# m-hamza-mughal/convofusion

Hardware: AMD Instinct MI355X
Metric: denoise-steps/sec (B=32 per GPU, 196-token latent, 1500 audio tokens, 1000-step DDPM schedule) (higher is better)
Workload: dtype f16x3 (fp16 hi/lo split operands, 3 MFMAs per product, f32 accumulate; f32-equivalent); fused cross-attention against the long (audio) memory: single-f16 operands (keys, values, queries, probabilities), f32 accumulate, in DDPM runs (operand policy 15; 1000-step DDPM golden at this shape: 2.3e-5 from; 1 GPU; configs[1]: B=32/GPU synthetic, L=196, S=(32, 1500, 32, 8, 1), 7-way guidance (denoiser batch 224), DDPM 1000-step schedule, 20 timed iterations of the hipGraph-captured loop; parallelism=batch-shard x1, one all_gather of latents

## Files before the change

convofusion_amd/csrc/attn_fused.hpp:

```cpp
#pragma once
#include "cfd_common.hpp"

struct SelfAttnArgs {
  const char* qk;
  const char* vts;
  char* o;
  int L, Lv;
};

#define SELF_ATTN_WAVES 8
#define SA_WAIT_VM_LGKM0(N) __builtin_amdgcn_s_waitcnt(((N) & 15) | 0x70 | ((((N) >> 4) & 3) << 14))
template <int CFD_KI = 0>
__global__ void __launch_bounds__(SELF_ATTN_WAVES * 64, 4) self_attn_fused_kernel(const SelfAttnArgs a) {
  extern __shared__ __attribute__((aligned(16))) char smem[];
  constexpr int STAGE = 32768, VOFF = 16384;
  const int lane = threadIdx.x & 63;
  const int wid = __builtin_amdgcn_readfirstlane(threadIdx.x >> 6);
  const int l15 = lane & 15, q4 = lane >> 4, sw = l15 >> 1;
  const int b = blockIdx.z, h = blockIdx.y;
  const int q = blockIdx.x * (SELF_ATTN_WAVES * 16) + wid * 16 + l15;
  const bool qvalid = q < a.L;
  const bool wave_active = (int)(blockIdx.x * (SELF_ATTN_WAVES * 16)) + wid * 16 < a.L;
  const int qc = qvalid ? q : a.L - 1;
  const long long ROW = 4096;

  const int cpos = lane & 7, rsub = lane >> 3;
  const int nkv = (a.L + 31) / 32;
  auto fill = [&](int kt) __attribute__((always_inline)) {
    char* st = smem + (kt & 1) * STAGE;
#pragma unroll
    for (int n = 0; n < 2; ++n) {
      const int g = wid + SELF_ATTN_WAVES * n, ks = g >> 2, rg = g & 3;
      const int r = rg * 8 + rsub;
      const int key = min(kt * 32 + r, a.L - 1);
      const char* src = a.qk + ((long long)b * a.L + key) * ROW + (long long)(16 + h * 4 + ks) * 128 + ((cpos ^ ((r >> 1) & 7)) << 4);
      __builtin_amdgcn_global_load_lds((gptr_t)src, (lptr_t)(st + ks * 4096 + rg * 1024), 16, 0, 0);
    }
#pragma unroll
    for (int n = 0; n < 2; ++n) {
      const int rg = wid + SELF_ATTN_WAVES * n;
      const int r = rg * 8 + rsub;
      const char* src = a.vts + ((long long)b * CFD_D + h * 128 + r) * ((long long)a.Lv * 4) + (long long)kt * 128 + ((cpos ^ ((r >> 1) & 7)) << 4);
      __builtin_amdgcn_global_load_lds((gptr_t)src, (lptr_t)(st + VOFF + rg * 1024), 16, 0, 0);
    }
  };
  fill(0);

  spx8 qh[4], ql[4];
  {
    const char* qp = a.qk + ((long long)b * a.L + qc) * ROW + (long long)(h * 4) * 128 + q4 * 16;
#pragma unroll
    for (int ks = 0; ks < 4; ++ks) {
      qh[ks] = *reinterpret_cast<const spx8*>(qp + ks * 128);
      ql[ks] = *reinterpret_cast<const spx8*>(qp + ks * 128 + 64);
    }
  }
  f32x4 o[8];
#pragma unroll
  for (int f = 0; f < 8; ++f) o[f] = f32x4{0.f, 0.f, 0.f, 0.f};
  float m = -INFINITY, lsum = 0.f, mc_run = -INFINITY;

  for (int kt = 0; kt < nkv; ++kt) {
    SA_WAIT_VM_LGKM0(0);
    __builtin_amdgcn_s_barrier();
    if (kt + 1 < nkv) fill(kt + 1);
    if (!wave_active) continue;
    const char* st = smem + (kt & 1) * STAGE;

    f32x4 s[2];
#pragma unroll
    for (int t = 0; t < 2; ++t) s[t] = f32x4{0.f, 0.f, 0.f, 0.f};
#pragma unroll
    for (int ks = 0; ks < 4; ++ks) {
#pragma unroll
      for (int t = 0; t < 2; ++t) {
        const char* kp = st + ks * 4096 + (t * 16 + l15) * 128;
        const spx8 xh = *reinterpret_cast<const spx8*>(kp + ((q4 ^ sw) << 4));
        const spx8 xl = *reinterpret_cast<const spx8*>(kp + (((4 + q4) ^ sw) << 4));
        s[t] = SP_MFMA(xl, qh[ks], s[t], 0, 0, 0);
        s[t] = SP_MFMA(xh, ql[ks], s[t], 0, 0, 0);
        s[t] = SP_MFMA(xh, qh[ks], s[t], 0, 0, 0);
      }
    }
// ... 3 lines not shown
#pragma unroll
    for (int e = 0; e < 8; ++e) {
      const int key = kt * 32 + 16 * (e >> 2) + 4 * q4 + (e & 3);
      p[e] = key < a.L ? s[e >> 2][e & 3] : -INFINITY;
      mx = fmaxf(mx, p[e]);
    }
    mx = xlane_max(mx);
    const float m_new = fmaxf(m, mx);
    const float mc = m_new * LOG2E;
    const float scale = __builtin_amdgcn_exp2f(mc_run - mc);
    mc_run = mc;
    float ps = 0.f;
#pragma unroll
    for (int e = 0; e < 8; ++e) {
      p[e] = __builtin_amdgcn_exp2f(fmaf(p[e], LOG2E, -mc));
      ps += p[e];
    }
    lsum = lsum * scale + xlane_sum(ps);
    m = m_new;
    if (!__all(scale == 1.0f)) {
#pragma unroll
      for (int f = 0; f < 8; ++f) { o[f][0] *= scale; o[f][1] *= scale; o[f][2] *= scale; o[f][3] *= scale; }
    }
    spx8 ph, pl;
#pragma unroll
    for (int e = 0; e < 8; ++e) {
      sp_t hi, lo;
      split_f32(p[e], hi, lo);
      ph[e] = hi;
      pl[e] = lo;
    }
#pragma unroll
    for (int f = 0; f < 8; ++f) {
      const char* vp = st + VOFF + (f * 16 + l15) * 128;
      const spx8 xh = *reinterpret_cast<const spx8*>(vp + ((q4 ^ sw) << 4));
      const spx8 xl = *reinterpret_cast<const spx8*>(vp + (((4 + q4) ^ sw) << 4));
      o[f] = SP_MFMA(xl, ph, o[f], 0, 0, 0);
      o[f] = SP_MFMA(xh, pl, o[f], 0, 0, 0);
      o[f] = SP_MFMA(xh, ph, o[f], 0, 0, 0);
    }
  }
  __syncthreads();
  {
    constexpr int RS = 64 * 4 + 16;
    char* strip = smem + wid * (16 * RS);
    const float inv = 1.0f / lsum;
#pragma unroll
    for (int half = 0; half < 2; ++half) {
#pragma unroll
      for (int f = 0; f < 4; ++f) {
        const f32x4 src = o[half * 4 + f];
        *reinterpret_cast<f32x4*>(strip + l15 * RS + (f * 16 + q4 * 4) * 4) = f32x4{src[0] * inv, src[1] * inv, src[2] * inv, src[3] * inv};
      }
      asm volatile("s_waitcnt lgkmcnt(0)" ::: "memory");
#pragma unroll
      for (int it = 0; it < 2; ++it) {
        const int row = it * 8 + (lane >> 3), c8 = (lane & 7) * 8;
        const int qq = blockIdx.x * (SELF_ATTN_WAVES * 16) + wid * 16 + row;
        const f32x4 v0 = *reinterpret_cast<const f32x4*>(strip + row * RS + c8 * 4);
        const f32x4 v1 = *reinterpret_cast<const f32x4*>(strip + row * RS + c8 * 4 + 16);
        if (qq < a.L) {
          const float v[8] = {v0[0], v0[1], v0[2], v0[3], v1[0], v1[1], v1[2], v1[3]};
          sp_store8(a.o + ((long long)b * a.L + qq) * (CFD_D * 4), h * 128 + half * 64 + c8, v);
        }
      }
      asm volatile("s_waitcnt lgkmcnt(0)" ::: "memory");
    }
  }
}
// ... 1 lines not shown
```

convofusion_amd/csrc/cfd_core.hip:

```cpp
#include "cfd_internal.hpp"

static thread_local char g_err[1024] = "";
int fail(int code, const char* fmt, ...) {
  va_list ap;
  va_start(ap, fmt);
  vsnprintf(g_err, sizeof(g_err), fmt, ap);
  va_end(ap);
  return code;
}

extern "C" const char* cfd_last_error(void) { return g_err; }

static long long env_int(const char* name, long long dflt) {
  const char* v = getenv(name);
  return v ? atoll(v) : dflt;
}

#ifndef CFD_SOURCE_HASH
#define CFD_SOURCE_HASH "unknown"
#endif
static const char g_source_hash[] = "cfd-src-hash:" CFD_SOURCE_HASH;
extern "C" const char* cfd_source_hash(void) { return g_source_hash + 13; }

extern "C" int cfd_create(const cfd_config* cfg, cfd_handle* out) {
// ... 36 lines not shown
  (void)hipEventCreate(&c->pev[0]);
  (void)hipEventCreate(&c->pev[1]);
  if (hipStreamCreateWithFlags(&c->own_stream, hipStreamNonBlocking) != hipSuccess) { delete c; return fail(CFD_E_HIP, "stream create"); }
  *out = c;
  return CFD_OK;
}

extern "C" void cfd_destroy(cfd_handle c) {
  if (!c) return;
  (void)hipSetDevice(c->cfg.device);
  (void)hipDeviceSynchronize();
  if (c->gexec) (void)hipGraphExecDestroy(c->gexec);
  if (c->graph) (void)hipGraphDestroy(c->graph);
  for (auto& wg : c->weg_graph) {
    if (wg.exec) (void)hipGraphExecDestroy(wg.exec);
    if (wg.graph) (void)hipGraphDestroy(wg.graph);
  }
  if (c->weg_ev) (void)hipEventDestroy(c->weg_ev);
  c->weg_io.release();
  c->weg_rt_ws.release();
  c->sat.release();
  c->acen.release();
  for (auto& kv : c->raw) kv.second.release();
  DBuf* all[] = {&c->we_sp, &c->wp_sp, &c->wp_f, &c->ln_cd_p, &c->we_all, &c->be_all, &c->tsin, &c->weg_ws, &c->weg_tok, &c->latents, &c->coef, &c->inoise, &c->hist, &c->wtab, &c->esrc, &c->enoise, &c->ekeep};
  for (DBuf* b : all) b->release();
  c->wk[0].release();
  c->wk[1].release();
  for (int j = 0; j < CFD_NMEM; ++j) {
    c->wk_all_sp[j].release(); c->wv_all_sp[j].release(); c->mem_own[j].release(); c->perm_map[j].release();
    c->lv_map[j].release(); c->lv_mask[j].release();
  }
  c->pic_s.release(); c->pic_part.release(); c->pic_err.release();
  for (auto& l : c->lw) {
    DBuf* lb[] = {&l.wqk_f, &l.wv_f, &l.w1_f, &l.ln_cd, &l.wqk_sp, &l.bqk, &l.wv_sp, &l.wo_sp, &l.bo2, &l.wtb1_sp, &l.wtb2_sp, &l.w1_sp, &l.w2_sp, &l.cross_bias};
    for (DBuf* b : lb) b->release();
  }
  if (c->own_stream) (void)hipStreamDestroy(c->own_stream);
  if (c->pev[0]) (void)hipEventDestroy(c->pev[0]);
  if (c->pev[1]) (void)hipEventDestroy(c->pev[1]);
  delete c;
}

extern "C" int cfd_load_tensor(cfd_handle c, const char* name, const float* data, size_t numel, int is_device) {
  if (!c || !name || !data || numel == 0) return fail(CFD_E_ARG, "null/empty argument");
  HIPCHK(hipSetDevice(c->cfg.device));
  DBuf& b = c->raw[name];
  CHK(b.ensure(numel * sizeof(float)));
  HIPCHK(hipMemcpy(b.p, data, numel * sizeof(float), is_device ? hipMemcpyDeviceToDevice : hipMemcpyHostToDevice));
  c->raw_numel[name] = numel;
  c->finalized = false;
  c->weg_sig.clear();
  return CFD_OK;
}

static int need(Ctx* c, const std::string& name, size_t numel, const float** out, bool at_least = false) {
  auto it = c->raw_numel.find(name);
  if (it == c->raw_numel.end()) return fail(CFD_E_STATE, "missing tensor '%s' (state-dict key denoiser.%s)", name.c_str(), name.c_str());
  if (at_least ? (it->second < numel || it->second % CFD_D) : (it->second != numel))
    return fail(CFD_E_SHAPE, "tensor '%s' has %zu elements, expected %s%zu", name.c_str(), it->second, at_least ? ">= " : "", numel);
  *out = c->raw[name].as<float>();
  return CFD_OK;
}

int to_sp(Ctx* c, const float* src, long long R, int K, DBuf& dst, long long dst_rows) {
  if (dst_rows < 0) dst_rows = R;
  CHK(dst.ensure((size_t)dst_rows * K * 4));
  if (dst_rows > R) HIPCHK(hipMemset(dst.p, 0, (size_t)dst_rows * K * 4));
// ... 64 lines not shown
  CHK(c->be_all.ensure((size_t)nl * 2 * 2 * D * 4));
  DBuf tmpf, tmpd1, tmpd2, vd1, vd2, accd, tmpfold;
  CHK(tmpf.ensure((size_t)3 * D * D * 4));
  CHK(tmpd1.ensure((size_t)D * D * 8));
  CHK(tmpd2.ensure((size_t)D * D * 8));
  CHK(vd1.ensure(D * 8));
  CHK(vd2.ensure(D * 8));
  CHK(accd.ensure(D * 8));
  const long long kfeat = (long long)nl * D;
  DBuf wk_f[CFD_NMEM], wv_f[CFD_NMEM];
  for (int j = 0; j < CFD_NMEM; ++j) {
    CHK(wk_f[j].ensure((size_t)(kfeat + 32) * D * 4));
    HIPCHK(hipMemset(wk_f[j].p, 0, (size_t)(kfeat + 32) * D * 4));
    CHK(wv_f[j].ensure((size_t)kfeat * D * 4));
  }
  const dim3 blk(256);
  auto grid1 = [](long long n) { return dim3((unsigned)((n + 255) / 256)); };

  for (int l = 0; l < nl; ++l) {
    LayerW& w = c->lw[l];
    const std::string p = "decoder.layers." + std::to_string(l) + ".";
    const float *ipw, *ipb, *ow, *ob;
    const float* ipw_self = nullptr;
    CHK(need(c, p + "self_attn.in_proj_weight", (size_t)3 * D * D, &ipw));
    ipw_self = ipw;
    CHK(need(c, p + "self_attn.in_proj_bias", 3 * D, &ipb));
    CHK(need(c, p + "self_attn.out_proj.weight", (size_t)D * D, &ow));
    CHK(need(c, p + "self_attn.out_proj.bias", D, &ob));
    const float qs = (float)std::sqrt(1.0 / (double)CFD_HD);
    float* tf = tmpf.as<float>();
    hipLaunchKernelGGL(scale_copy_kernel<>, grid1((long long)D * D), blk, 0, 0, ipw, tf, (long long)D * D, qs);
    hipLaunchKernelGGL(scale_copy_kernel<>, grid1((long long)D * D), blk, 0, 0, ipw + (size_t)D * D, tf + (size_t)D * D,
                       (long long)D * D, 1.0f);
    CHK(to_sp(c, tf, 2 * D, D, w.wqk_sp));
    CHK(w.bqk.ensure(2 * D * 4));
    hipLaunchKernelGGL(scale_copy_kernel<>, grid1(D), blk, 0, 0, ipb, w.bqk.as<float>(), (long long)D, qs);
    hipLaunchKernelGGL(scale_copy_kernel<>, grid1(D), blk, 0, 0, ipb + D, w.bqk.as<float>() + D, (long long)D, 1.0f);
    CHK(to_sp(c, ipw + (size_t)2 * D * D, D, D, w.wv_sp));
    CHK(to_sp(c, ow, D, D, w.wo_sp));
    CHK(w.bo2.ensure(D * 4));
    hipLaunchKernelGGL((fold_mv_kernel<float, float, float>), grid1(D), blk, 0, 0, ow, (long long)D, 1LL, ipb + 2 * D,
                       (const double*)nullptr, ob, w.bo2.as<float>(), D, D, 1.0, (const float*)nullptr);
    for (int tb = 0; tb < 2; ++tb) {
      const std::string q = p + (tb == 0 ? "time_block1." : "time_block2.");
      CHK(need(c, q + "emb_layers.1.weight", (size_t)2 * D * D, &t0));
      HIPCHK(hipMemcpy(c->we_all.as<float>() + ((size_t)(2 * l + tb) * 2 * D) * D, t0, (size_t)2 * D * D * 4, hipMemcpyDeviceToDevice));
      CHK(need(c, q + "emb_layers.1.bias", 2 * D, &t0));
      HIPCHK(hipMemcpy(c->be_all.as<float>() + (size_t)(2 * l + tb) * 2 * D, t0, (size_t)2 * D * 4, hipMemcpyDeviceToDevice));
      CHK(need(c, q + "out_layers.2.weight", (size_t)D * D, &t0));
      CHK(to_sp(c, t0, D, D, tb == 0 ? w.wtb1_sp : w.wtb2_sp));
      CHK(need(c, q + "norm.weight", D, tb == 0 ? &w.tb1g : &w.tb2g));
      CHK(need(c, q + "norm.bias", D, tb == 0 ? &w.tb1b : &w.tb2b));
      CHK(need(c, q + "out_layers.2.bias", D, tb == 0 ? &w.btb1 : &w.btb2));
    }
    CHK(need(c, p + "norm1.weight", D, &w.ln1g)); CHK(need(c, p + "norm1.bias", D, &w.ln1b));
    CHK(need(c, p + "norm2.weight", D, &w.ln2g)); CHK(need(c, p + "norm2.bias", D, &w.ln2b));
    CHK(need(c, p + "norm3.weight", D, &w.ln3g)); CHK(need(c, p + "norm3.bias", D, &w.ln3b));
    CHK(need(c, p + "linear1.weight", (size_t)CFD_FF * D, &t0)); CHK(to_sp(c, t0, CFD_FF, D, w.w1_sp));
    CHK(need(c, p + "linear1.bias", CFD_FF, &w.b1));
    {
      CHK(w.ln_cd.ensure(6144 * 4));
      float* cd = w.ln_cd.as<float>();
      CHK(ln_fold_weight(c, tmpf.as<float>(), 2 * D, D, w.ln1g, w.ln1b, tmpfold, w.wqk_f, cd, cd + 1024));
      CHK(ln_fold_weight(c, ipw_self + (size_t)2 * D * D, D, D, w.ln1g, w.ln1b, tmpfold, w.wv_f, cd + 2048, cd + 2560));
      CHK(ln_fold_weight(c, t0, CFD_FF, D, w.ln3g, w.ln3b, tmpfold, w.w1_f, cd + 3072, cd + 4096));
    }
    CHK(need(c, p + "linear2.weight", (size_t)D * CFD_FF, &t0)); CHK(to_sp(c, t0, D, CFD_FF, w.w2_sp));
    CHK(need(c, p + "linear2.bias", D, &w.b2));
    const float *fw, *fb;
    CHK(need(c, p + "att_fuser.weight", (size_t)D * 5 * D, &fw));
    CHK(need(c, p + "att_fuser.bias", D, &fb));
// ... 67 lines not shown
```

convofusion_amd/csrc/cfd_forward.hip:

```cpp
#include "cfd_internal.hpp"



int enqueue_denoise(Ctx* c, hipStream_t st) {
  CHK(enqueue_memside(c, st));
  if (c->w->pb.rt) return enqueue_rows_rt(c, st);
  return enqueue_rows(c, st, 0, c->w->pb.Be);
}


int enqueue_rows_rt(Ctx* c, hipStream_t st, const RtSave* sv) {
  const Problem& p = c->w->pb;
  const int nl = c->nl, L = p.L, tpr = (L + 15) / 16, ntile = p.Be * tpr;
  const int* dstep = c->w->d_step.as<int>();
  const int lds_xpv = (p.Sp_tot / 32) * 2048 + 8 * (p.Sp_tot <= 512 ? 2 : 4) * 2048 + 16 * 32 * 16 + 512 + 2048;
#define RT_SET_LDS(kernel, bytes) HIPCHK(hipFuncSetAttribute(reinterpret_cast<const void*>(&kernel), hipFuncAttributeMaxDynamicSharedMemorySize, bytes))
  static unsigned long long attr = 0;
  if (!((attr >> (c->cfg.device & 63)) & 1ull)) {
    RT_SET_LDS((rt_gemm_kernel<RT_PRO_SP, RT_EPI_EMBED, 256, CFD_LAT / 32, 1>), rt_gemm_lds(RT_PRO_SP, 256, CFD_LAT / 32, 1));
    RT_SET_LDS((rt_gemm_kernel<RT_PRO_LN, RT_EPI_QKV, 512, CFD_D / 32, 3>), rt_gemm_lds(RT_PRO_LN, 512, CFD_D / 32, 3));
    RT_SET_LDS((rt_gemm_kernel<RT_PRO_SP, RT_EPI_RESID, 256, CFD_D / 32, 1>), rt_gemm_lds(RT_PRO_SP, 256, CFD_D / 32, 1));
    RT_SET_LDS((rt_gemm_kernel<RT_PRO_ADALN, RT_EPI_RESID, 512, CFD_D / 32, 1>), rt_gemm_lds(RT_PRO_ADALN, 512, CFD_D / 32, 1));
    RT_SET_LDS((rt_gemm_kernel<RT_PRO_LN, RT_EPI_SPLIT, 512, CFD_D / 32, 2>), rt_gemm_lds(RT_PRO_LN, 512, CFD_D / 32, 2));
    RT_SET_LDS((rt_gemm_kernel<RT_PRO_SP, RT_EPI_RESID, 512, CFD_FF / 32, 1>), rt_gemm_lds(RT_PRO_SP, 512, CFD_FF / 32, 1));
// ... 46 lines not shown
    if (_e != hipSuccess) return fail(CFD_E_HIP, "row-tile launch failed: %s", hipGetErrorString(_e));          \
  } while (0)
  {
    RtGemmArgs a = base;
    a.a_sp = c->w->sample_sp.as<char>(); a.w = c->we_sp.as<char>(); a.bias = rawp(c, "latent_embd.bias");
    a.bh = rawp(c, "bh_embedding.weight"); a.qpe = rawp(c, "query_pos.pe"); a.xo = X(0, 0);
    RT_LAUNCH(CFD_PROF_GEMM_TOKEN, RT_PRO_SP, RT_EPI_EMBED, 256, CFD_LAT / 32, 1, CFD_D, a);
  }
  if (c->stop_stage == 1) return CFD_OK;
  auto time_block = [&](const DBuf& w, const float* g, const float* b, const float* bias, int tbidx, const float* xin, float* xout) -> int {
    RtGemmArgs a = base;
    a.x = xin; a.xr = xin; a.xo = xout;
    a.g = g; a.b = b; a.ss = ss_now + (size_t)tbidx * 2 * CFD_D; a.w = w.as<char>(); a.bias = bias;
    if (nfb2) RT_LAUNCH(CFD_PROF_GEMM_TOKEN, RT_PRO_ADALN, RT_EPI_RESID, 512, CFD_D / 32, 2, CFD_D, a);
    else RT_LAUNCH(CFD_PROF_GEMM_TOKEN, RT_PRO_ADALN, RT_EPI_RESID, 512, CFD_D / 32, 1, CFD_D, a);
    return CFD_OK;
  };
  RtXArgs xa;
  memset(&xa, 0, sizeof(xa));
  xa.L = L; xa.tpr = tpr; xa.nl = nl; xa.Sp_tot = p.Sp_tot; xa.rsp = c->w->p_sp.as<float>();
  int nkb = 0;
  for (int j = 0; j < CFD_NMEM; ++j) {
    xa.map[j] = p.map[j]; xa.rows[j] = p.U[j] * p.Sp[j]; xa.S[j] = p.S[j]; xa.Sp[j] = p.Sp[j]; xa.off[j] = p.off[j];
    xa.cbt[j] = cbt_now[j]; xa.att[j] = p.att[j]; xa.att_slot[j] = p.att_slot[j];
    memcpy(xa.inst[j], p.rt_inst[j], RT_ARG_ROWS);
    xa.blk0[j] = nkb; nkb += p.Sp[j] / 16;
  }
  xa.blk0[CFD_NMEM] = nkb;
  xa.att_b0 = p.att_nb > 0 ? p.att_b0 : 0;
  xa.att_nb = p.att_nb > 0 ? p.att_nb : p.Be;
  xa.att_step = p.att_nb > 0 ? c->w->d_step.as<int>() : nullptr;
  for (int l = 0; l < nl; ++l) {
    const LayerW& w = c->lw[l];
    char* qk = sv ? sv->qk[l] : c->w->qk_sp.as<char>();
    char* vt = sv ? sv->vt[l] : c->w->rt_vt.as<char>();
    {
      RtGemmArgs a = base;
      a.x = X(l, 0);
      a.g = w.ln1g; a.b = w.ln1b; a.w = w.wqk_sp.as<char>(); a.w2 = w.wv_sp.as<char>(); a.nfb_qk = 2 * CFD_D / 16;
      a.bias = w.bqk.as<float>(); a.o_sp = qk; a.ld_o = 2 * CFD_D * 4; a.vt = vt;
      RT_LAUNCH(CFD_PROF_GEMM_TOKEN, RT_PRO_LN, RT_EPI_QKV, 512, CFD_D / 32, 3, 3 * CFD_D, a);
    }
    {
      RtSelfArgs a{qk, vt, c->w->o_sp.as<char>(), L, tpr};
      Bracket br(c, CFD_PROF_GEMM_ATTN, st);
      hipLaunchKernelGGL(rt_selfattn_kernel<>, dim3(CFD_NHEAD, ntile), dim3(256), 40960, st, a);
      HIPCHK(hipGetLastError());
    }
    {
      RtGemmArgs a = base;
      a.xr = X(l, 0); a.xo = X(l, 1);
      a.a_sp = c->w->o_sp.as<char>(); a.w = w.wo_sp.as<char>(); a.bias = w.bo2.as<float>();
      if (nfb2) RT_LAUNCH(CFD_PROF_GEMM_TOKEN, RT_PRO_SP, RT_EPI_RESID, 256, CFD_D / 32, 2, CFD_D, a);
      else RT_LAUNCH(CFD_PROF_GEMM_TOKEN, RT_PRO_SP, RT_EPI_RESID, 256, CFD_D / 32, 1, CFD_D, a);
    }
    if (c->stop_stage == 2 + 4 * l) return CFD_OK;
    CHK(time_block(w.wtb1_sp, w.tb1g, w.tb1b, w.btb1, 2 * l, X(l, 1), X(l, 2)));
    if (c->stop_stage == 3 + 4 * l) {
      if (!sv) HIPCHK(hipMemcpyAsync(xw, hw, (size_t)p.M * CFD_D * 4, hipMemcpyDeviceToDevice, st));
      return CFD_OK;
    }
    {
      RtXArgs a = xa;
      a.x = X(l, 2); a.xo = X(l, 3);
      a.sc = sv ? sv->sc[l] : c->w->sc.as<float>();
      a.cst = sv ? sv->cst[l] : c->w->ssc.as<float>();
      a.ln_g = w.ln2g; a.ln_b = w.ln2b; a.bias = w.cross_bias.as<float>(); a.layer = l;
      for (int j = 0; j < CFD_NMEM; ++j) {
        const size_t rows = (size_t)p.U[j] * p.Sp[j];
        a.K[j] = c->w->kall_sp[j].as<char>() + (size_t)l * rows * CFD_D * 4;
        a.VT[j] = c->w->vt_all[j].as<char>() + (size_t)l * rows * CFD_D * 4;
        a.kb[j] = kb_now[j] + (size_t)l * CFD_D;
// ... 113 lines not shown
  auto token_gemm_resid_ln = [&](const DBuf& w, int K, const char* y, const float* bias, long long rows, const float* g, const float* b,
                                 int adaln, int tbidx) -> int {
    CHK(token_gemm_resid(w, K, y, bias, rows));
    return ln(g, b, adaln, tbidx, c->w->h_sp.as<char>(), rows);
  };
  const bool ln_fold = c->ln_fold != 0 && L == 16 && !c->stop_stage && row0 == 0 && Be == p.Be &&
                       (c->ln_fold > 0 || (M >= 512 && M <= 3840));
  if (ln_fold) CHK(c->w->ln_stat.ensure((size_t)M * LN_SLOTS * 2 * 4));
  auto token_gemm_resid_stat = [&](const DBuf& w, int K, const char* y, const float* bias, long long rows, char* xs) -> int {
    GemmArgs a = gemm_args();
    a.X[0] = w.as<char>(); a.ldx[0] = (long long)K * 4; a.I[0] = CFD_D; a.Iclamp[0] = CFD_D; a.kt[0] = K / 32;
    a.Y = y; a.ldy = (long long)K * 4; a.J = (int)rows; a.Jclamp = (int)rows;
    EpiResidStat e{c->w->x.as<float>(), 0, bias, xs, c->w->ln_stat.as<float>()};
    return run_gemm_midsize<MODE_PLAIN>(c, CFD_PROF_GEMM_TOKEN, a, e, st);
  };
  bool h_raw = false;
  static unsigned long long attr = 0;
  if (!((attr >> (c->cfg.device & 63)) & 1ull)) {
    HIPCHK(hipFuncSetAttribute(reinterpret_cast<const void*>(&self_attn_fused_kernel<>), hipFuncAttributeMaxDynamicSharedMemorySize, 65536));
    HIPCHK(hipFuncSetAttribute(reinterpret_cast<const void*>(&xattn_fused_kernel<false, false>), hipFuncAttributeMaxDynamicSharedMemorySize, XA_LDS));
    HIPCHK(hipFuncSetAttribute(reinterpret_cast<const void*>(&xattn_fused_kernel<false, true>), hipFuncAttributeMaxDynamicSharedMemorySize, XA_LDS));
    HIPCHK(hipFuncSetAttribute(reinterpret_cast<const void*>(&xattn_fused_kernel<true, false>), hipFuncAttributeMaxDynamicSharedMemorySize, XA_LDS));
    attr |= 1ull << (c->cfg.device & 63);
  }

  bool h_ready = false;
  for (int l = 0; l < nl; ++l) {
    const LayerW& w = c->lw[l];
    const int Ba = (l == 0) ? Bs : Be;
    const long long Ma = (long long)Ba * L;
    if (!h_ready) CHK(ln(w.ln1g, w.ln1b, 0, 0, c->w->h_sp.as<char>(), Ma));
    h_ready = false;
    bool qkv_one_launch = false;
    const int Lv = (L + 31) / 32 * 32;
    {
      GemmArgs a = gemm_args();
      a.X[0] = w.wqk_sp.as<char>(); a.ldx[0] = ROWB; a.I[0] = 2 * CFD_D; a.Iclamp[0] = 2 * CFD_D; a.kt[0] = CFD_D / 32;
      a.Y = c->w->h_sp.as<char>(); a.ldy = ROWB; a.J = (int)Ma; a.Jclamp = (int)Ma;
      EpiSplit e{c->w->qk_sp.as<char>(), 2 * ROWB, 0, 0, w.bqk.as<float>(), 0, 0};
      GemmArgs av = gemm_args();
      av.X[0] = c->w->h_sp.as<char>(); av.ldx[0] = ROWB; av.xbs[0] = (long long)L * ROWB; av.I[0] = Lv; av.Iclamp[0] = L; av.kt[0] = CFD_D / 32;
      av.Y = w.wv_sp.as<char>(); av.ldy = ROWB; av.J = CFD_D; av.Jclamp = CFD_D;
      EpiSplit ev{c->w->vts_sp.as<char>(), (long long)Lv * 4, (long long)CFD_D * Lv * 4, 0, nullptr, 0, 1};
      if (L == 16) {
        GemmArgs ag = a;
        ag.nslot = 2;
        ag.X[1] = w.wv_sp.as<char>(); ag.ldx[1] = ROWB; ag.I[1] = CFD_D; ag.Iclamp[1] = CFD_D; ag.kt[1] = CFD_D / 32;
        EpiQkvT eg{c->w->qk_sp.as<char>(), 2 * ROWB, w.bqk.as<float>(), c->w->vts_sp.as<char>(), 1};
        if (h_raw) {
          EpiLn<EpiQkvT> el;
          static_cast<EpiQkvT&>(el) = eg;
          const float* cd = w.ln_cd.as<float>();
          el.ln_stat = c->w->ln_stat.as<float>(); el.ln_c[0] = cd; el.ln_d[0] = cd + 1024; el.ln_c[1] = cd + 2048; el.ln_d[1] = cd + 2560; el.ln_eps = 1e-5f;
          ag.X[0] = w.wqk_f.as<char>(); ag.X[1] = w.wv_f.as<char>();
          CHK((run_gemm_midsize<MODE_GROUPED>(c, CFD_PROF_GEMM_TOKEN, ag, el, st)));
        } else
        CHK((run_gemm<MODE_GROUPED>(c, CFD_PROF_GEMM_TOKEN, ag, eg, 1, 1, st)));
        qkv_one_launch = true;
      } else {
      CHK((run_gemm<MODE_PLAIN>(c, CFD_PROF_GEMM_TOKEN, a, e, 1, 1, st)));
      CHK((run_gemm<MODE_PLAIN>(c, CFD_PROF_GEMM_TOKEN, av, ev, Ba, 1, st)));
      }
    }
    if (qkv_one_launch) {
      RtSelfArgs a{c->w->qk_sp.as<char>(), c->w->vts_sp.as<char>(), c->w->o_sp.as<char>(), L, 1};
      Bracket br(c, CFD_PROF_GEMM_ATTN, st);
      hipLaunchKernelGGL(rt_selfattn_kernel<>, dim3(CFD_NHEAD, Ba), dim3(256), 40 * 1024, st, a);
      HIPCHK(hipGetLastError());
    } else {
      SelfAttnArgs a{c->w->qk_sp.as<char>(), c->w->vts_sp.as<char>(), c->w->o_sp.as<char>(), L, Lv};
      Bracket br(c, CFD_PROF_GEMM_ATTN, st);
      hipLaunchKernelGGL(self_attn_fused_kernel<>, dim3((L + SELF_ATTN_WAVES * 16 - 1) / (SELF_ATTN_WAVES * 16), CFD_NHEAD, Ba), dim3(SELF_ATTN_WAVES * 64), 65536, st, a);
      HIPCHK(hipGetLastError());
    }
    CHK(token_gemm_resid_ln(w.wo_sp, CFD_D, c->w->o_sp.as<char>(), w.bo2.as<float>(), Ma, w.tb1g, w.tb1b, 1, 2 * l));
    if (c->stop_stage == 2 + 4 * l) return CFD_OK;
    CHK(token_gemm_resid(w.wtb1_sp, CFD_D, c->w->h_sp.as<char>(), w.btb1, Ma));
    if (c->stop_stage == 3 + 4 * l) return CFD_OK;
    if (Ma != M) {
      const long long n4 = Ma * (CFD_D / 4);
      LAUNCH(CFD_PROF_ROWS, replicate_rows_kernel<>, dim3((unsigned)((n4 + 255) / 256)), blk, st, reinterpret_cast<float4*>(c->w->x.as<float>()), n4,
             (int)(M / Ma));
    }
    if (fused_x) {
      XAttnArgs a;
      memset(&a, 0, sizeof(a));
      a.x = c->w->x.as<float>(); a.ln_g = w.ln2g; a.ln_b = w.ln2b; a.bias = w.cross_bias.as<float>(); a.L = L;
      for (int j = 0; j < CFD_NMEM; ++j) {
        const size_t rows = (size_t)p.U[j] * p.Sp[j];
        const bool f16 = p.xa_f16 && ((p.xa_f16_mask >> j) & 1);
        a.K[j] = f16 ? c->w->k16[j].as<char>() + (size_t)l * rows * 1024 : c->w->kall_sp[j].as<char>() + (size_t)l * rows * ROWB;
        a.cb[j] = c->w->cb[j].as<float>() + (size_t)l * rows;
        a.VT[j] = f16 ? c->w->v16[j].as<char>() + (size_t)l * rows * 1024 : c->w->vt_all[j].as<char>() + (size_t)l * rows * ROWB;
        a.Sp[j] = p.Sp[j];
        const bool stat = (p.static_mask >> j) & 1;
        a.rs_off[j] = (unsigned)((size_t)(nl - l) * rows * 4);
        a.kb[j] = stat ? kb_now[j] + (size_t)l * CFD_D : c->w->zeros512.as<float>();
        a.kb_stride[j] = stat ? nl * CFD_D + 32 : 0;
        a.vb[j] = stat ? vb_now[j] + (size_t)l * CFD_D : c->w->zeros512.as<float>();
        a.vb_stride[j] = stat ? nl * CFD_D : 0;
      }
      a.d_step = rows_now ? nullptr : dstep;
      a.one_j = -1;
// ... 449 lines not shown
```

convofusion_amd/csrc/cfd_internal.hpp:

```cpp
#pragma once
#include <hip/hip_runtime.h>

#include <cmath>
#include <cstdarg>
#include <cstdio>
#include <cstdlib>
#include <cstring>
#include <algorithm>
#include <map>
#include <string>
#include <vector>

#include "../../include/cfdenoise.h"
#include "../../include/cfdenoise_dev.h"
#include "gemm_sp.hpp"
#include "rows.hpp"
#include "attn_fused.hpp"
#include "xattn_fused.hpp"
#include "rowtile.hpp"


int fail(int code, const char* fmt, ...);
#define HIPCHK(expr)                                                                               \
  do {                                                                                             \
    hipError_t _e = (expr);                                                                        \
    if (_e != hipSuccess) return fail(CFD_E_HIP, "%s failed: %s (%s:%d)", #expr, hipGetErrorString(_e), __FILE__, __LINE__); \
  } while (0)
#define CHK(expr)            \
  do {                       \
    int _r = (expr);         \
    if (_r != CFD_OK) return _r; \
  } while (0)

static const char* MEM_NAMES[CFD_NMEM] = {"spkemb", "alsn", "tlsn", "apb", "lsnemb"};

struct DBuf {
  void* p = nullptr;
  size_t bytes = 0;
  int ensure(size_t n) {
    if (n <= bytes) return CFD_OK;
    if (p) (void)hipFree(p);
    p = nullptr;
    bytes = 0;
    HIPCHK(hipMalloc(&p, n));
    bytes = n;
    return CFD_OK;
  }
  void release() {
    if (p) (void)hipFree(p);
    p = nullptr;
    bytes = 0;
  }
  template <class T> T* as() const { return reinterpret_cast<T*>(p); }
};

struct LayerW {
  DBuf wqk_sp, bqk, wv_sp, wo_sp, bo2, wtb1_sp, wtb2_sp, w1_sp, w2_sp, cross_bias;
  DBuf wqk_f, wv_f, w1_f, ln_cd;
  const float *ln1g, *ln1b, *tb1g, *tb1b, *btb1, *ln2g, *ln2b, *tb2g, *tb2b, *btb2, *ln3g, *ln3b, *b1, *b2;
};

struct Problem {
  int Be = 0, L = 0, Lp = 0;
  long long M = 0;
  int U[CFD_NMEM], S[CFD_NMEM], Sp[CFD_NMEM], off[CFD_NMEM], Sp_tot = 0;
  const float* mem[CFD_NMEM];
  const int* map[CFD_NMEM];
  const uint8_t* mask[CFD_NMEM];
  int has_mask[CFD_NMEM];
  float* att[CFD_NMEM];
  int att_b0 = 0, att_nb = 0;
  bool prev_same = false;
  bool att_fused = false;
  long long att_slot[CFD_NMEM] = {0, 0, 0, 0, 0};
  int tmode = 0;
  int lv_rows = 0, lv_i0 = 0, lv_U[CFD_NMEM] = {0, 0, 0, 0, 0};
  int share_B = 0;
  int T = 1;
  int jbig = -1, nruns = 0, nlong = 0, nshort = 0;
  int run_row0[8], run_len[8], run_u[8];
  int xa_nwg = 0;
  int xa0_nwg_a = 0, xa0_nwg_b = 0;
  bool xa_flush = false;
  int xa_one = -1;
  bool xa_f16 = false;
  int xa_f16_mask = 0;
  int static_mask = 0;
  bool rt = false;
  int rt_use_inst = 0;
  unsigned char rt_inst[CFD_NMEM][RT_ARG_ROWS];
};

struct RtSave {
  float* x[CFD_MAX_LAYERS + 1][5];
  char* qk[CFD_MAX_LAYERS];
  char* vt[CFD_MAX_LAYERS];
  float* sc[CFD_MAX_LAYERS];
  float* cst[CFD_MAX_LAYERS];
  float* pre[CFD_MAX_LAYERS];
};

struct WegRtState {
  std::vector<long long> sig;
  RtSave sv;
  float *att = nullptr, *d_att = nullptr, *fws = nullptr, *dP = nullptr, *G[3] = {nullptr, nullptr, nullptr}, *dz = nullptr, *dy = nullptr,
        *dh = nullptr, *dO = nullptr, *dqkv = nullptr;
  int launches = 0;
  int T = 1;
  int stop = 0, stop_gi = -1;
  int B = 0, L = 0, Sp_tot = 0, St = 0;
  int dy_keys = 0, focus_large = 0;
};

struct Work {
  Problem pb;
  DBuf x, h_sp, qk_sp, vts_sp, ssc, sp_sp, o_sp, u_sp, sc, p_sp, eps, sample_sp;
  DBuf ln_stat;
  DBuf n_sp[CFD_NMEM], kall_sp[CFD_NMEM], cb[CFD_NMEM], vt_all[CFD_NMEM];
  DBuf temb_tab, h1_tab, ss_tab, trows, iota, long_rows, short_rows, zero_mask;
  DBuf ca[CFD_NMEM], asq[CFD_NMEM], kbtab[CFD_NMEM], vbtab[CFD_NMEM], b_tab, b_sp, bsq, zeros512;
  DBuf xa_wgs, xa_segs, xa_stamps, xa0_wgs_a, xa0_segs_a, xa0_wgs_b, xa0_segs_b, xa_dedup, xa_one_va, xa_att_raw, xa_att_mc, xa_att_fin, xa_att_desc;
  DBuf d_step;
  bool fwd_mem_valid = false;
  int fwd_U[CFD_NMEM] = {0, 0, 0, 0, 0}, fwd_S[CFD_NMEM] = {0, 0, 0, 0, 0}, fwd_Be = 0, fwd_L = 0;
  bool fwd_att = false;
  bool fwd_mask[CFD_NMEM] = {false, false, false, false, false}, fwd_map[CFD_NMEM] = {false, false, false, false, false};
  unsigned long long fwd_wver = 0;
  DBuf rt_vt, rt_cbt[CFD_NMEM];
  DBuf k16[CFD_NMEM], v16[CFD_NMEM];
  DBuf rt_cur;
  std::vector<int32_t> tt_key;
  long long tt_wver = -1;
  int tt_mem_mask = 0;
  const float* now_ss = nullptr;
  const float* now_kb[CFD_NMEM] = {nullptr, nullptr, nullptr, nullptr, nullptr};
  const float* now_vb[CFD_NMEM] = {nullptr, nullptr, nullptr, nullptr, nullptr};
  void release() {
    DBuf* all[] = {&x, &h_sp, &qk_sp, &vts_sp, &ssc, &sp_sp, &o_sp, &u_sp, &sc, &p_sp, &eps, &sample_sp, &temb_tab, &h1_tab, &ss_tab, &trows, &iota,
                   &long_rows, &short_rows, &zero_mask, &ln_stat, &b_tab, &b_sp, &bsq, &zeros512, &xa_wgs, &xa_segs, &xa_stamps, &xa0_wgs_a, &xa0_segs_a, &xa0_wgs_b, &xa0_segs_b, &xa_dedup, &xa_one_va, &xa_att_raw, &xa_att_mc, &xa_att_fin, &xa_att_desc, &d_step, &rt_vt, &rt_cur};
    for (DBuf* b : all) b->release();
    for (int j = 0; j < CFD_NMEM; ++j) {
      n_sp[j].release(); kall_sp[j].release(); cb[j].release(); vt_all[j].release(); ca[j].release(); asq[j].release(); kbtab[j].release();
      vbtab[j].release(); rt_cbt[j].release(); k16[j].release(); v16[j].release();
    }
  }
};

struct RunMode {
  bool weighted = false;
  int k0 = 0;
  bool edit = false;
  float* traj = nullptr;
  bool anchor = false;
  const float* anchor_ring = nullptr;
  int anchor_n = 0;
  bool tie = false;
  bool tie_final = false;
  bool replay = false;
};

struct cfd_handle_s {
  cfd_config cfg;
  int nl = 0;
  bool finalized = false;
  std::map<std::string, DBuf> raw;
  std::map<std::string, size_t> raw_numel;
  DBuf we_sp, wp_sp, we_all, be_all;
  DBuf wp_f, ln_cd_p;
  DBuf wk_all_sp[CFD_NMEM], wv_all_sp[CFD_NMEM];
  std::vector<LayerW> lw;
  int qpe_rows = 0, mpe_rows = 0;
// ... 213 lines not shown
```

convofusion_amd/csrc/cfd_problem.hip:

```cpp
#include "cfd_internal.hpp"

struct XaRow {
  int xrow;
  int inst[CFD_NMEM];
  int aux;
  int one;
  int att;
};

static void make_xattn_worklist(const Problem& p, const std::vector<XaRow>& rows, int mem_mask, std::vector<XaWg>& wgs, std::vector<XaSeg>& segs,
                                size_t& n_active, bool& has_flush) {
  const int L = p.L, nqt = (L + 15) / 16;
  wgs.clear(); segs.clear(); n_active = 0;
  int order[CFD_NMEM], n_mem = 0, n_online = 0;
  for (int j = 0; j < CFD_NMEM; ++j)
    if ((mem_mask >> j) & 1) order[n_mem++] = j;
  if (n_mem == 0 || rows.empty()) return;
  std::stable_sort(order, order + n_mem, [&](int a, int b) { return p.Sp[a] > p.Sp[b]; });
  for (int oi = 0; oi < n_mem; ++oi) n_online += p.Sp[order[oi]] > XA_KEYS;
  const int jg = order[0];
  std::vector<int> inst_group(p.U[jg], -1);
  std::vector<std::vector<int>> groups;
  for (size_t r = 0; r < rows.size(); ++r) {
    int& g = inst_group[rows[r].inst[jg]];
// ... 287 lines not shown
        if (!srows.empty()) HIPCHK(hipMemcpy(c->w->short_rows.p, srows.data(), srows.size() * 4, hipMemcpyHostToDevice));
      }
    }
  }
  p.rt = c->rt_on && tmode == 0 && L <= RT_MAX_L && p.M <= c->rt_max_rows && p.Sp_tot <= RT_MAX_KEYS;
  if (p.rt) {
    if (!keep_lists) p.rt_use_inst = Be <= RT_ARG_ROWS;
    for (int j = 0; j < CFD_NMEM && p.rt_use_inst && !keep_lists; ++j) {
      std::vector<int> hm(Be);
      if (mem[j].row_map) HIPCHK(hipMemcpy(hm.data(), mem[j].row_map, (size_t)Be * 4, hipMemcpyDeviceToHost));
      else for (int b = 0; b < Be; ++b) hm[b] = b;
      for (int b = 0; b < Be; ++b) {
        if (hm[b] < 0 || hm[b] >= p.U[j]) return fail(CFD_E_ARG, "memory %s: row_map[%d] = %d outside [0, %d)", MEM_NAMES[j], b, hm[b], p.U[j]);
        if (hm[b] > 255) p.rt_use_inst = 0;
        p.rt_inst[j][b] = (unsigned char)hm[b];
      }
    }
    CHK(c->w->rt_vt.ensure((size_t)Be * CFD_D * RT_MAX_L * 4));
    HIPCHK(hipMemset(c->w->rt_vt.p, 0, (size_t)Be * CFD_D * RT_MAX_L * 4));
  }
  {
    bool any_att = false;
    for (int j = 0; j < CFD_NMEM; ++j) any_att = any_att || p.att[j];
    p.att_fused = any_att && !p.rt && tmode == 0 && c->fused_xattn;
    if (p.att_fused) { p.att_b0 = 0; p.att_nb = Be; }
  }
  if (!keep_lists) CHK(build_xattn_worklist(c, mem, true));
  if (p.att_fused && p.xa_nwg <= 0) { p.att_fused = false; p.att_nb = 0; }
  if (p.att_fused && !keep_lists) CHK(setup_att_fused(c));
  const long long M = p.M;
  const int nl = c->nl;
  CHK(c->w->x.ensure((size_t)M * CFD_D * 4));
  CHK(c->w->h_sp.ensure((size_t)M * CFD_D * 4));
  CHK(c->w->qk_sp.ensure((size_t)M * 2 * CFD_D * 4));
  CHK(c->w->vts_sp.ensure((size_t)Be * CFD_D * ((L + 63) / 64 * 64) * 4));
  CHK(c->w->ssc.ensure((size_t)Be * CFD_NHEAD * L * p.Lp * 4));
  CHK(c->w->sp_sp.ensure((size_t)Be * CFD_NHEAD * L * p.Lp * 4));
  CHK(c->w->o_sp.ensure((size_t)M * CFD_D * 4));
  CHK(c->w->u_sp.ensure((size_t)M * CFD_FF * 4));
  CHK(c->w->sc.ensure((size_t)M * p.Sp_tot * 4));
  CHK(c->w->p_sp.ensure((size_t)M * p.Sp_tot * 4));
  CHK(c->w->eps.ensure((size_t)M * CFD_LAT * 4));
  CHK(c->w->sample_sp.ensure((size_t)M * CFD_LAT * 4));
  for (int j = 0; j < CFD_NMEM; ++j) {
    const size_t rows = (size_t)p.U[j] * p.Sp[j];
    CHK(c->w->n_sp[j].ensure(rows * CFD_D * 4));
    CHK(c->w->kall_sp[j].ensure(rows * nl * CFD_D * 4));
    CHK(c->w->cb[j].ensure(rows * (nl + 1) * 4));
    CHK(c->w->vt_all[j].ensure(rows * nl * CFD_D * 4));
  }
  if (c->w->temb_tab.bytes < (size_t)T * CFD_D * 4 || c->w->ss_tab.bytes < (size_t)T * nl * 2 * 2 * CFD_D * 4) {
    c->w->tt_key.clear();
    c->w->tt_mem_mask = 0;
  }
  CHK(c->w->temb_tab.ensure((size_t)T * CFD_D * 4));
  CHK(c->w->h1_tab.ensure((size_t)T * CFD_D * 4));
  CHK(c->w->ss_tab.ensure((size_t)T * nl * 2 * 2 * CFD_D * 4));
  CHK(c->w->trows.ensure((size_t)T * 4));
  return CFD_OK;
}

int build_time_tables(Ctx* c, const int32_t* trows_host, int T, hipStream_t st) {
  for (int i = 0; i < T; ++i)
    if (trows_host[i] < 0 || trows_host[i] >= c->tsin_rows)
      return fail(CFD_E_ARG, "timestep %d outside the sinusoid table (0..%d)", trows_host[i], c->tsin_rows - 1);
  HIPCHK(hipMemcpyAsync(c->w->trows.p, trows_host, (size_t)T * 4, hipMemcpyHostToDevice, st));
  Work* w = c->w;
  const bool same = w->tt_wver == c->wver && (int)w->tt_key.size() == T && std::equal(w->tt_key.begin(), w->tt_key.end(), trows_host);
// ... 208 lines not shown
```

Baseline: 83.78 denoise-steps/s (32-utterance batches, summed over GPUs).

## Fuse V projection into QKV GEMM and read V via LDS transpose loads

Concatenates the Q, K and V projection weights into one weight so the token GEMM produces Q, K and V in a single row-major buffer. This removes the separate batched V-transpose GEMM launch. The self-attention kernel now loads V rows directly from that buffer and uses ds_read_tr16_b64 transpose reads from LDS to build the MFMA fragments. The cost is more complex swizzled LDS addressing and a wider QKV output row stride.

New measurement: 85.06 denoise-steps/s (32-utterance batches, summed over GPUs) (median of 6 runs). 1.02x the previous value.

```diff
diff --git a/convofusion_amd/csrc/attn_fused.hpp b/convofusion_amd/csrc/attn_fused.hpp
--- a/convofusion_amd/csrc/attn_fused.hpp
+++ b/convofusion_amd/csrc/attn_fused.hpp
@@ -2,11 +2,21 @@
 #include "cfd_common.hpp"
 
 struct SelfAttnArgs {
-  const char* qk;
-  const char* vts;
+  const char* qkv;
   char* o;
-  int L, Lv;
+  long long ldq;
+  int L;
 };
+
+typedef __fp16 sa_tr4 __attribute__((__vector_size__(4 * sizeof(__fp16))));
+__device__ __forceinline__ spx8 sa_tr_frag(const char* p) {
+  const sa_tr4 a = __builtin_amdgcn_ds_read_tr16_b64_v4f16((__attribute__((address_space(3))) sa_tr4*)(lptr_t)p);
+  const sa_tr4 b = __builtin_amdgcn_ds_read_tr16_b64_v4f16((__attribute__((address_space(3))) sa_tr4*)(lptr_t)(p + 2048));
+  spx8 r;
+#pragma unroll
+  for (int e = 0; e < 4; ++e) { r[e] = (sp_t)a[e]; r[4 + e] = (sp_t)b[e]; }
+  return r;
+}
 
 #define SELF_ATTN_WAVES 8
 #define SA_WAIT_VM_LGKM0(N) __builtin_amdgcn_s_waitcnt(((N) & 15) | 0x70 | ((((N) >> 4) & 3) << 14))
@@ -22,10 +32,11 @@
   const bool qvalid = q < a.L;
   const bool wave_active = (int)(blockIdx.x * (SELF_ATTN_WAVES * 16)) + wid * 16 < a.L;
   const int qc = qvalid ? q : a.L - 1;
-  const long long ROW = 4096;
+  const long long ROW = a.ldq;
 
   const int cpos = lane & 7, rsub = lane >> 3;
   const int nkv = (a.L + 31) / 32;
+  const int vpl = lane >> 5, vr = (lane >> 2) & 7, vch = vpl * 4 + ((((lane >> 1) & 1) ^ (vr >> 2)) << 1) + (lane & 1);
   auto fill = [&](int kt) __attribute__((always_inline)) {
     char* st = smem + (kt & 1) * STAGE;
 #pragma unroll
@@ -33,22 +44,22 @@
       const int g = wid + SELF_ATTN_WAVES * n, ks = g >> 2, rg = g & 3;
       const int r = rg * 8 + rsub;
       const int key = min(kt * 32 + r, a.L - 1);
-      const char* src = a.qk + ((long long)b * a.L + key) * ROW + (long long)(16 + h * 4 + ks) * 128 + ((cpos ^ ((r >> 1) & 7)) << 4);
+      const char* src = a.qkv + ((long long)b * a.L + key) * ROW + (long long)(16 + h * 4 + ks) * 128 + ((cpos ^ ((r >> 1) & 7)) << 4);
       __builtin_amdgcn_global_load_lds((gptr_t)src, (lptr_t)(st + ks * 4096 + rg * 1024), 16, 0, 0);
     }
 #pragma unroll
     for (int n = 0; n < 2; ++n) {
-      const int rg = wid + SELF_ATTN_WAVES * n;
-      const int r = rg * 8 + rsub;
-      const char* src = a.vts + ((long long)b * CFD_D + h * 128 + r) * ((long long)a.Lv * 4) + (long long)kt * 128 + ((cpos ^ ((r >> 1) & 7)) << 4);
-      __builtin_amdgcn_global_load_lds((gptr_t)src, (lptr_t)(st + VOFF + rg * 1024), 16, 0, 0);
+      const int g = wid + SELF_ATTN_WAVES * n, ks = g >> 2, rg = g & 3;
+      const int key = min(kt * 32 + rg * 8 + vr, a.L - 1);
+      const char* src = a.qkv + ((long long)b * a.L + key) * ROW + (long long)(32 + h * 4 + ks) * 128 + (vch << 4);
+      __builtin_amdgcn_global_load_lds((gptr_t)src, (lptr_t)(st + VOFF + g * 1024), 16, 0, 0);
     }
   };
   fill(0);
 
   spx8 qh[4], ql[4];
   {
-    const char* qp = a.qk + ((long long)b * a.L + qc) * ROW + (long long)(h * 4) * 128 + q4 * 16;
+    const char* qp = a.qkv + ((long long)b * a.L + qc) * ROW + (long long)(h * 4) * 128 + q4 * 16;
 #pragma unroll
     for (int ks = 0; ks < 4; ++ks) {
       qh[ks] = *reinterpret_cast<const spx8*>(qp + ks * 128);
@@ -118,9 +129,9 @@
     }
 #pragma unroll
     for (int f = 0; f < 8; ++f) {
-      const char* vp = st + VOFF + (f * 16 + l15) * 128;
-      const spx8 xh = *reinterpret_cast<const spx8*>(vp + ((q4 ^ sw) << 4));
-      const spx8 xl = *reinterpret_cast<const spx8*>(vp + (((4 + q4) ^ sw) << 4));
+      const char* vp = st + VOFF + (f >> 1) * 4096 + (q4 >> 1) * 1024 + ((q4 & 1) * 4 + (l15 >> 2)) * 64 + (((f & 1) ^ (q4 & 1)) << 5) + (l15 & 3) * 8;
+      const spx8 xh = sa_tr_frag(vp);
+      const spx8 xl = sa_tr_frag(vp + 512);
       o[f] = SP_MFMA(xl, ph, o[f], 0, 0, 0);
       o[f] = SP_MFMA(xh, pl, o[f], 0, 0, 0);
       o[f] = SP_MFMA(xh, ph, o[f], 0, 0, 0);
diff --git a/convofusion_amd/csrc/cfd_core.hip b/convofusion_amd/csrc/cfd_core.hip
--- a/convofusion_amd/csrc/cfd_core.hip
+++ b/convofusion_amd/csrc/cfd_core.hip
@@ -92,7 +92,7 @@
   }
   c->pic_s.release(); c->pic_part.release(); c->pic_err.release();
   for (auto& l : c->lw) {
-    DBuf* lb[] = {&l.wqk_f, &l.wv_f, &l.w1_f, &l.ln_cd, &l.wqk_sp, &l.bqk, &l.wv_sp, &l.wo_sp, &l.bo2, &l.wtb1_sp, &l.wtb2_sp, &l.w1_sp, &l.w2_sp, &l.cross_bias};
+    DBuf* lb[] = {&l.wqk_f, &l.wv_f, &l.w1_f, &l.ln_cd, &l.wqkv_sp, &l.bqk, &l.wo_sp, &l.bo2, &l.wtb1_sp, &l.wtb2_sp, &l.w1_sp, &l.w2_sp, &l.cross_bias};
     for (DBuf* b : lb) b->release();
   }
   if (c->own_stream) (void)hipStreamDestroy(c->own_stream);
@@ -223,11 +223,12 @@
     hipLaunchKernelGGL(scale_copy_kernel<>, grid1((long long)D * D), blk, 0, 0, ipw, tf, (long long)D * D, qs);
     hipLaunchKernelGGL(scale_copy_kernel<>, grid1((long long)D * D), blk, 0, 0, ipw + (size_t)D * D, tf + (size_t)D * D,
                        (long long)D * D, 1.0f);
-    CHK(to_sp(c, tf, 2 * D, D, w.wqk_sp));
-    CHK(w.bqk.ensure(2 * D * 4));
+    HIPCHK(hipMemcpy(tf + (size_t)2 * D * D, ipw + (size_t)2 * D * D, (size_t)D * D * 4, hipMemcpyDeviceToDevice));
+    CHK(to_sp(c, tf, 3 * D, D, w.wqkv_sp));
+    CHK(w.bqk.ensure(3 * D * 4));
+    HIPCHK(hipMemset(w.bqk.as<float>() + 2 * D, 0, D * 4));
     hipLaunchKernelGGL(scale_copy_kernel<>, grid1(D), blk, 0, 0, ipb, w.bqk.as<float>(), (long long)D, qs);
     hipLaunchKernelGGL(scale_copy_kernel<>, grid1(D), blk, 0, 0, ipb + D, w.bqk.as<float>() + D, (long long)D, 1.0f);
-    CHK(to_sp(c, ipw + (size_t)2 * D * D, D, D, w.wv_sp));
     CHK(to_sp(c, ow, D, D, w.wo_sp));
     CHK(w.bo2.ensure(D * 4));
     hipLaunchKernelGGL((fold_mv_kernel<float, float, float>), grid1(D), blk, 0, 0, ow, (long long)D, 1LL, ipb + 2 * D,
diff --git a/convofusion_amd/csrc/cfd_forward.hip b/convofusion_amd/csrc/cfd_forward.hip
--- a/convofusion_amd/csrc/cfd_forward.hip
+++ b/convofusion_amd/csrc/cfd_forward.hip
@@ -102,12 +102,12 @@
   xa.att_step = p.att_nb > 0 ? c->w->d_step.as<int>() : nullptr;
   for (int l = 0; l < nl; ++l) {
     const LayerW& w = c->lw[l];
-    char* qk = sv ? sv->qk[l] : c->w->qk_sp.as<char>();
+    char* qk = sv ? sv->qk[l] : c->w->qkv_sp.as<char>();
     char* vt = sv ? sv->vt[l] : c->w->rt_vt.as<char>();
     {
       RtGemmArgs a = base;
       a.x = X(l, 0);
-      a.g = w.ln1g; a.b = w.ln1b; a.w = w.wqk_sp.as<char>(); a.w2 = w.wv_sp.as<char>(); a.nfb_qk = 2 * CFD_D / 16;
+      a.g = w.ln1g; a.b = w.ln1b; a.w = w.wqkv_sp.as<char>(); a.w2 = w.wqkv_sp.as<char>() + (size_t)2 * CFD_D * CFD_D * 4; a.nfb_qk = 2 * CFD_D / 16;
       a.bias = w.bqk.as<float>(); a.o_sp = qk; a.ld_o = 2 * CFD_D * 4; a.vt = vt;
       RT_LAUNCH(CFD_PROF_GEMM_TOKEN, RT_PRO_LN, RT_EPI_QKV, 512, CFD_D / 32, 3, 3 * CFD_D, a);
     }
@@ -287,21 +287,17 @@
     if (!h_ready) CHK(ln(w.ln1g, w.ln1b, 0, 0, c->w->h_sp.as<char>(), Ma));
     h_ready = false;
     bool qkv_one_launch = false;
-    const int Lv = (L + 31) / 32 * 32;
     {
       GemmArgs a = gemm_args();
-      a.X[0] = w.wqk_sp.as<char>(); a.ldx[0] = ROWB; a.I[0] = 2 * CFD_D; a.Iclamp[0] = 2 * CFD_D; a.kt[0] = CFD_D / 32;
+      a.X[0] = w.wqkv_sp.as<char>(); a.ldx[0] = ROWB; a.I[0] = 3 * CFD_D; a.Iclamp[0] = 3 * CFD_D; a.kt[0] = CFD_D / 32;
       a.Y = c->w->h_sp.as<char>(); a.ldy = ROWB; a.J = (int)Ma; a.Jclamp = (int)Ma;
-      EpiSplit e{c->w->qk_sp.as<char>(), 2 * ROWB, 0, 0, w.bqk.as<float>(), 0, 0};
-      GemmArgs av = gemm_args();
-      av.X[0] = c->w->h_sp.as<char>(); av.ldx[0] = ROWB; av.xbs[0] = (long long)L * ROWB; av.I[0] = Lv; av.Iclamp[0] = L; av.kt[0] = CFD_D / 32;
-      av.Y = w.wv_sp.as<char>(); av.ldy = ROWB; av.J = CFD_D; av.Jclamp = CFD_D;
-      EpiSplit ev{c->w->vts_sp.as<char>(), (long long)Lv * 4, (long long)CFD_D * Lv * 4, 0, nullptr, 0, 1};
+      EpiSplit e{c->w->qkv_sp.as<char>(), 3 * ROWB, 0, 0, w.bqk.as<float>(), 0, 0};
       if (L == 16) {
         GemmArgs ag = a;
         ag.nslot = 2;
-        ag.X[1] = w.wv_sp.as<char>(); ag.ldx[1] = ROWB; ag.I[1] = CFD_D; ag.Iclamp[1] = CFD_D; ag.kt[1] = CFD_D / 32;
-        EpiQkvT eg{c->w->qk_sp.as<char>(), 2 * ROWB, w.bqk.as<float>(), c->w->vts_sp.as<char>(), 1};
+        ag.I[0] = 2 * CFD_D; ag.Iclamp[0] = 2 * CFD_D;
+        ag.X[1] = w.wqkv_sp.as<char>() + 2 * CFD_D * ROWB; ag.ldx[1] = ROWB; ag.I[1] = CFD_D; ag.Iclamp[1] = CFD_D; ag.kt[1] = CFD_D / 32;
+        EpiQkvT eg{c->w->qkv_sp.as<char>(), 2 * ROWB, w.bqk.as<float>(), c->w->vts_sp.as<char>(), 1};
         if (h_raw) {
           EpiLn<EpiQkvT> el;
           static_cast<EpiQkvT&>(el) = eg;
@@ -314,16 +310,15 @@
         qkv_one_launch = true;
       } else {
       CHK((run_gemm<MODE_PLAIN>(c, CFD_PROF_GEMM_TOKEN, a, e, 1, 1, st)));
-      CHK((run_gemm<MODE_PLAIN>(c, CFD_PROF_GEMM_TOKEN, av, ev, Ba, 1, st)));
       }
     }
     if (qkv_one_launch) {
-      RtSelfArgs a{c->w->qk_sp.as<char>(), c->w->vts_sp.as<char>(), c->w->o_sp.as<char>(), L, 1};
+      RtSelfArgs a{c->w->qkv_sp.as<char>(), c->w->vts_sp.as<char>(), c->w->o_sp.as<char>(), L, 1};
       Bracket br(c, CFD_PROF_GEMM_ATTN, st);
       hipLaunchKernelGGL(rt_selfattn_kernel<>, dim3(CFD_NHEAD, Ba), dim3(256), 40 * 1024, st, a);
       HIPCHK(hipGetLastError());
     } else {
-      SelfAttnArgs a{c->w->qk_sp.as<char>(), c->w->vts_sp.as<char>(), c->w->o_sp.as<char>(), L, Lv};
+      SelfAttnArgs a{c->w->qkv_sp.as<char>(), c->w->o_sp.as<char>(), 3 * ROWB, L};
       Bracket br(c, CFD_PROF_GEMM_ATTN, st);
       hipLaunchKernelGGL(self_attn_fused_kernel<>, dim3((L + SELF_ATTN_WAVES * 16 - 1) / (SELF_ATTN_WAVES * 16), CFD_NHEAD, Ba), dim3(SELF_ATTN_WAVES * 64), 65536, st, a);
       HIPCHK(hipGetLastError());
diff --git a/convofusion_amd/csrc/cfd_internal.hpp b/convofusion_amd/csrc/cfd_internal.hpp
--- a/convofusion_amd/csrc/cfd_internal.hpp
+++ b/convofusion_amd/csrc/cfd_internal.hpp
@@ -55,7 +55,7 @@
 };
 
 struct LayerW {
-  DBuf wqk_sp, bqk, wv_sp, wo_sp, bo2, wtb1_sp, wtb2_sp, w1_sp, w2_sp, cross_bias;
+  DBuf wqkv_sp, bqk, wo_sp, bo2, wtb1_sp, wtb2_sp, w1_sp, w2_sp, cross_bias;
   DBuf wqk_f, wv_f, w1_f, ln_cd;
   const float *ln1g, *ln1b, *tb1g, *tb1b, *btb1, *ln2g, *ln2b, *tb2g, *tb2b, *btb2, *ln3g, *ln3b, *b1, *b2;
 };
@@ -114,7 +114,7 @@
 
 struct Work {
   Problem pb;
-  DBuf x, h_sp, qk_sp, vts_sp, ssc, sp_sp, o_sp, u_sp, sc, p_sp, eps, sample_sp;
+  DBuf x, h_sp, qkv_sp, vts_sp, ssc, sp_sp, o_sp, u_sp, sc, p_sp, eps, sample_sp;
   DBuf ln_stat;
   DBuf n_sp[CFD_NMEM], kall_sp[CFD_NMEM], cb[CFD_NMEM], vt_all[CFD_NMEM];
   DBuf temb_tab, h1_tab, ss_tab, trows, iota, long_rows, short_rows, zero_mask;
@@ -136,7 +136,7 @@
   const float* now_kb[CFD_NMEM] = {nullptr, nullptr, nullptr, nullptr, nullptr};
   const float* now_vb[CFD_NMEM] = {nullptr, nullptr, nullptr, nullptr, nullptr};
   void release() {
-    DBuf* all[] = {&x, &h_sp, &qk_sp, &vts_sp, &ssc, &sp_sp, &o_sp, &u_sp, &sc, &p_sp, &eps, &sample_sp, &temb_tab, &h1_tab, &ss_tab, &trows, &iota,
+    DBuf* all[] = {&x, &h_sp, &qkv_sp, &vts_sp, &ssc, &sp_sp, &o_sp, &u_sp, &sc, &p_sp, &eps, &sample_sp, &temb_tab, &h1_tab, &ss_tab, &trows, &iota,
                    &long_rows, &short_rows, &zero_mask, &ln_stat, &b_tab, &b_sp, &bsq, &zeros512, &xa_wgs, &xa_segs, &xa_stamps, &xa0_wgs_a, &xa0_segs_a, &xa0_wgs_b, &xa0_segs_b, &xa_dedup, &xa_one_va, &xa_att_raw, &xa_att_mc, &xa_att_fin, &xa_att_desc, &d_step, &rt_vt, &rt_cur};
     for (DBuf* b : all) b->release();
     for (int j = 0; j < CFD_NMEM; ++j) {
diff --git a/convofusion_amd/csrc/cfd_problem.hip b/convofusion_amd/csrc/cfd_problem.hip
--- a/convofusion_amd/csrc/cfd_problem.hip
+++ b/convofusion_amd/csrc/cfd_problem.hip
@@ -343,8 +343,8 @@
   const int nl = c->nl;
   CHK(c->w->x.ensure((size_t)M * CFD_D * 4));
   CHK(c->w->h_sp.ensure((size_t)M * CFD_D * 4));
-  CHK(c->w->qk_sp.ensure((size_t)M * 2 * CFD_D * 4));
-  CHK(c->w->vts_sp.ensure((size_t)Be * CFD_D * ((L + 63) / 64 * 64) * 4));
+  CHK(c->w->qkv_sp.ensure((size_t)M * (L == 16 ? 2 : 3) * CFD_D * 4));
+  if (L == 16) CHK(c->w->vts_sp.ensure((size_t)Be * CFD_D * 64 * 4));
   CHK(c->w->ssc.ensure((size_t)Be * CFD_NHEAD * L * p.Lp * 4));
   CHK(c->w->sp_sp.ensure((size_t)Be * CFD_NHEAD * L * p.Lp * 4));
   CHK(c->w->o_sp.ensure((size_t)M * CFD_D * 4));
```
